# NethermindEth/zinc

Hardware: AMD Instinct MI355X
Metric: Zip commit+open MCoeffs/s at 2^24 witness (higher is better)
Workload: dtype i64

## Files before the change

zinc_amd/csrc/kernels_commit.cuh:

```cuda
#pragma once
#include <hip/hip_runtime.h>
#include <stdint.h>

#include "blake3.cuh"

namespace zipk {

typedef __int128 i128;
typedef unsigned __int128 u128;

#ifdef ZIPK_DEBUG_STAMPS
constexpr uint32_t kStampRec = 64;
__device__ __forceinline__ unsigned long long stamp_hw_id() {
    const uint32_t xcc = __builtin_amdgcn_s_getreg((3 << 11) | 20), hw = __builtin_amdgcn_s_getreg((31 << 11) | 4);
    return (unsigned long long)xcc | ((unsigned long long)hw << 8);
}
#endif

struct CommitArgs {
    const int64_t *evals;
    const uint32_t *perm1;
    const uint32_t *perm2;
    uint64_t *rows;
    uint32_t compact_rows;
// ... 121 lines not shown
    static constexpr bool MASKED = MODE != kStoreAll;
    uint32_t w0[E], w1[E], w2[E];
    const uint64_t *lz_lo = nullptr;
    const uint32_t *lz_hi = nullptr;
    uint32_t lz_stride = 0;
    template <int E0>
    __device__ __forceinline__ void entry(uint32_t &a, uint32_t &b, uint32_t &c) const {
        if (LAZY) {
            const uint64_t lo = lz_lo[E0 * lz_stride];
            a = (uint32_t)lo;
            b = (uint32_t)(lo >> 32);
            c = lz_hi[E0 * lz_stride];
        } else {
            a = w0[E0];
            b = w1[E0];
            c = w2[E0];
        }
    }
    uint64_t *out_row;
    uint32_t *tree;
    uint32_t cw, T, tid;
    uint32_t base = 0;
    uint32_t compact = 0;
    uint32_t smask = 0xFFFFFFFFu;
    static constexpr uint32_t NW = MODE == kStorePacked ? 32u : 8u;
    uint8_t *pk_v = nullptr, *pk_n = nullptr;
    uint32_t pk_off0 = 0, pk_off1 = 0, pk_off2 = 0;
    __device__ __forceinline__ void set_packed(const CommitArgs &a, uint32_t row) {
        uint8_t *g = a.pk + (size_t)(row >> 2) * 4 * a.pk_stride;
        pk_v = g + (row & 3u) * 16u;
        pk_n = g + (row & 3u) * 32u;
        pk_off0 = 4u * a.pk_off0;
        pk_off1 = 4u * a.pk_off1;
        pk_off2 = 4u * a.pk_off2;
    }
    uint32_t ptab[16] = {};
    template <int K>
    __device__ __forceinline__ uint32_t pbase() const { return (ptab[K >> 1] >> ((K & 1) * 16)) & 0xFFFFu; }
    static __device__ __forceinline__ uint32_t lanes_below(uint64_t m) {
        return __builtin_amdgcn_mbcnt_hi((uint32_t)(m >> 32), __builtin_amdgcn_mbcnt_lo((uint32_t)m, 0u));
    }
    template <int E0>
    __device__ __forceinline__ void store_row_of(uint32_t d0, uint32_t d1, uint32_t d2) {
        if (MASKED && !(smask & (1u << E0))) return;
        const uint32_t j = base + E0 * T + tid;
        const uint32_t s = (uint32_t)((int32_t)d2 >> 31);
        if (MODE == kStorePacked) {
            const uint32_t pos = pbase<E0>() + lanes_below(__builtin_amdgcn_ballot_w64(true));
            *reinterpret_cast<uint4 *>(pk_v + (size_t)pos * 64) = make_uint4(d0, d1, d2, s);
        } else if (compact) {
            *reinterpret_cast<uint4 *>(out_row + (size_t)j * 2) = make_uint4(d0, d1, d2, s);
        } else {
            uint4 *o = reinterpret_cast<uint4 *>(out_row + (size_t)j * 4);
            o[0] = make_uint4(d0, d1, d2, s);
            o[1] = make_uint4(s, s, s, s);
        }
    }
    template <int E0>
    __device__ __forceinline__ void store_row() {
        uint32_t d0, d1, d2;
        entry<E0>(d0, d1, d2);
        store_row_of<E0>(d0, d1, d2);
    }
    template <int E0>
    __device__ __forceinline__ void leaf(uint32_t (&h)[8]) {
        uint32_t d0, d1, d2;
        entry<E0>(d0, d1, d2);
        store_row_of<E0>(d0, d1, d2);
        blake3_leaf_sext96(d0, d1, d2, h);
        if (!MASKED || (smask & (0x100u << E0))) {
            if (MODE == kStorePacked) {
                const uint32_t pos = pbase<8 + E0>() + lanes_below(__builtin_amdgcn_ballot_w64(true));
                store_hash(reinterpret_cast<uint32_t *>(pk_n + pk_off0) + (size_t)pos * 32, h);
            } else {
                store_hash(tree + (size_t)(base + E0 * T + tid) * 8, h);
            }
        }
    }
    template <int LVL, int E0>
    __device__ __forceinline__ void store(const uint32_t (&h)[8]) {
        if (MASKED && LVL <= 2 && !(smask & ((LVL == 1 ? 0x10000u : 0x1000000u) << (E0 >> LVL)))) return;
        const uint32_t e = E0 + (tid & ((1u << LVL) - 1u));
        const uint32_t n = (base + e * T + tid) >> LVL;
        if (MODE == kStorePacked && LVL == 1) {
            const uint64_t act = __builtin_amdgcn_ballot_w64(true);
            const bool odd = tid & 1u;
            const uint32_t pos = (odd ? pbase<16 + (E0 >> 1) * 2 + 1>() : pbase<16 + (E0 >> 1) * 2>()) +
                                 lanes_below(act & (odd ? 0xAAAAAAAAAAAAAAAAull : 0x5555555555555555ull));
            store_hash(reinterpret_cast<uint32_t *>(pk_n + pk_off1) + (size_t)pos * 32, h);
        } else if (MODE == kStorePacked && LVL == 2) {
            const uint64_t act = __builtin_amdgcn_ballot_w64(true);
            const uint32_t q = tid & 3u;
            constexpr int K0 = 24 + ((E0 >> 2) & 1) * 4;
            const uint32_t b01 = (q & 1u) ? pbase<K0 + 1>() : pbase<K0>(), b23 = (q & 1u) ? pbase<K0 + 3>() : pbase<K0 + 2>();
            const uint32_t pos = ((q & 2u) ? b23 : b01) + lanes_below(act & (0x1111111111111111ull << q));
            store_hash(reinterpret_cast<uint32_t *>(pk_n + pk_off2) + (size_t)pos * 32, h);
        } else {
            store_hash(tree + ((size_t)level_off(cw, LVL) + n) * NW, h);
        }
    }
};

template <int E>
__device__ __forceinline__ uint32_t store_mask(const uint32_t *need, uint32_t cw, uint32_t base, uint32_t T, uint32_t tid) {
    if (!need) return 0xFFFFFFFFu;
    const uint32_t *nv = need, *n0 = nv + (cw + 31) / 32, *n1 = n0 + (cw + 31) / 32, *n2 = n1 + (cw / 2 + 31) / 32;
    uint32_t m = 0;
#pragma unroll
    for (int e = 0; e < E; e++) {
        const uint32_t j = base + e * T + tid;
        m |= ((nv[j >> 5] >> (j & 31)) & 1u) << e;
        m |= ((n0[j >> 5] >> (j & 31)) & 1u) << (8 + e);
    }
#pragma unroll
    for (int g = 0; g < E / 2; g++) {
        const uint32_t i = (base + (2 * g + (tid & 1u)) * T + tid) >> 1;
        m |= ((n1[i >> 5] >> (i & 31)) & 1u) << (16 + g);
    }
#pragma unroll
    for (int g = 0; g < E / 4; g++) {
        const uint32_t i = (base + (4 * g + (tid & 3u)) * T + tid) >> 2;
        m |= ((n2[i >> 5] >> (i & 31)) & 1u) << (24 + g);
    }
    return m;
}

template <int E, int E0, class Src>
__device__ __forceinline__ void store_rows_only(Src &src) {
    if constexpr (E0 < E) {
        src.template store_row<E0>();
        store_rows_only<E, E0 + 1>(src);
    }
}

template <int LVL, int E0, class Src>
__device__ __forceinline__ void bfly_hash(Src &src, uint32_t (&h)[8]) {
    if constexpr (LVL == 0) {
        src.template leaf<E0>(h);
    } else {
        uint32_t A[8], B[8], m[16];
        bfly_hash<LVL - 1, E0>(src, A);
        bfly_hash<LVL - 1, E0 + (1 << (LVL - 1))>(src, B);
        const bool up = (src.tid >> (LVL - 1)) & 1;
#pragma unroll
        for (int i = 0; i < 8; i++) {
            const uint32_t snd = up ? A[i] : B[i];
            const uint32_t rcv = __shfl_xor(snd, 1 << (LVL - 1), 64);
            m[i] = up ? rcv : A[i];
            m[8 + i] = up ? B[i] : rcv;
        }
        blake3_block64(m, h);
        src.template store<LVL, E0>(h);
    }
}

template <bool ILV>
__device__ __forceinline__ void upper_stage(const CommitArgs &a, uint32_t first, uint32_t nrows_c, uint32_t lvl, uint32_t nl,
                                            uint32_t lane, uint32_t nlanes) {
    constexpr uint32_t NW = kNodeWords<ILV>;
    const uint32_t cw = a.cw, depth = 31u - __builtin_clz(cw);
    const uint32_t u_shift = depth - (lvl - 1u) - nl;
    const uint32_t total = nrows_c << u_shift;
    const uint32_t slot0 = round_slot(blockIdx.x, gridDim.x, a.classes);
    for (uint32_t idx = lane; idx < total; idx += nlanes) {
        const uint32_t ri = idx >> u_shift, i = idx & ((1u << u_shift) - 1u);
        const uint32_t r = slot0 + (first + ri) * gridDim.x;
        uint32_t *tree = tree_of<ILV>(a.layers, cw, r);
        const uint32_t *ch = tree + ((size_t)level_off(cw, lvl - 1u) + ((size_t)i << nl)) * NW;
        uint32_t c0[8], c1[8], h0[8];
        load_hash(ch, c0);
        load_hash(ch + NW, c1);
        if (nl == 1u) {
            blake3_node(c0, c1, h0);
            store_hash(tree + ((size_t)level_off(cw, lvl) + i) * NW, h0);
            if (lvl == depth) store_hash(a.roots + (size_t)r * 8, h0);
        } else {
            uint32_t c2[8], c3[8], h1[8], h2[8];
            blake3_node(c0, c1, h0);
            uint32_t *o = tree + ((size_t)level_off(cw, lvl) + 2u * i) * NW;
            store_hash(o, h0);
            asm volatile("" ::: "memory");
            load_hash(ch + 2 * NW, c2);
            load_hash(ch + 3 * NW, c3);
            blake3_node(c2, c3, h1);
            store_hash(o + NW, h1);
            blake3_node(h0, h1, h2);
            store_hash(tree + ((size_t)level_off(cw, lvl + 1u) + i) * NW, h2);
            if (lvl + 1u == depth) store_hash(a.roots + (size_t)r * 8, h2);
        }
    }
}

struct ChunkCursor {
    uint32_t first = 0, index = 0;
    __device__ __forceinline__ bool ends_with(const CommitArgs &a, uint32_t round, bool last) const {
        if (last) return true;
        if (a.chunk_ends) return (a.chunk_ends >> round) & 1u;
        return (round + 1) % a.rounds_per_chunk == 0;
    }
    __device__ __forceinline__ void advance(uint32_t round) {
        first = round + 1;
        index++;
    }
};

constexpr uint32_t kFinisherFlagWords = 16;

template <bool HASH, bool ILV = false>
struct ChunkFinisher {
    bool pending = false;
    uint32_t p_first = 0, p_nrows = 0, p_lvl = 0, p_index = 0;
    uint32_t p_base = 0;
    uint32_t n_deferred = 0;
    uint32_t *flags = nullptr;

    __device__ __forceinline__ void init(uint32_t *lds_flags, uint32_t tid) {
        flags = lds_flags;
        if (tid < kFinisherFlagWords) lds_flags[tid] = 0;
    }

    __device__ __forceinline__ void top_of_row() const {
        if (HASH && pending) asm volatile("s_waitcnt vmcnt(0)" ::: "memory");
    }

    static __device__ __forceinline__ void publish(const CommitArgs &a, uint32_t index, uint32_t lane) {
        if (!a.chunk_done) return;
        asm volatile("s_waitcnt vmcnt(0)" ::: "memory");
        if (lane == 0) {
            __builtin_amdgcn_fence(__ATOMIC_RELEASE, "agent");
            asm volatile("s_waitcnt vmcnt(0)" ::: "memory");
            __hip_atomic_fetch_add(&a.chunk_done[index], 1u, __ATOMIC_RELAXED, __HIP_MEMORY_SCOPE_AGENT);
        }
    }

    static __device__ __forceinline__ void signal(uint32_t *flag, uint32_t lane) {
        asm volatile("s_waitcnt vmcnt(0)" ::: "memory");
        if (lane == 0) __hip_atomic_fetch_add(flag, 1u, __ATOMIC_RELEASE, __HIP_MEMORY_SCOPE_WORKGROUP);
    }
    static __device__ __forceinline__ void wait_for(uint32_t *flag, uint32_t target) {
        uint32_t spins = 0;
        while (__hip_atomic_load(flag, __ATOMIC_ACQUIRE, __HIP_MEMORY_SCOPE_WORKGROUP) < target) {
            __builtin_amdgcn_s_sleep(2);
            if (++spins > (1u << 24)) __builtin_trap();
        }
    }

    static __device__ __forceinline__ bool stage_wide(uint32_t cw, uint32_t lvl, uint32_t nl, uint32_t j) {
        return j == 0u || (cw >> (lvl - 1u + nl)) >= 64u;
    }
    static __device__ __forceinline__ uint32_t stage_waves(uint32_t cw, uint32_t depth, uint32_t lvl0, uint32_t j, uint32_t W) {
        const uint32_t lvl = lvl0 + 2u * j;
        if (lvl > depth) return 0u;
        return stage_wide(cw, lvl, depth - lvl >= 1u ? 2u : 1u, j) ? W : 1u;
    }
    __device__ __forceinline__ uint32_t target(uint32_t cw, uint32_t depth, uint32_t j, uint32_t W) const {
        return (n_deferred - 1u) * stage_waves(cw, depth, p_base, j, W) + stage_waves(cw, depth, p_lvl, j, W);
    }
    __device__ __forceinline__ void after_hash(const CommitArgs &a, uint32_t wave, uint32_t lane, uint32_t T) {
        if (!(HASH && pending)) return;
        pending = false;
        n_deferred++;
        constexpr uint32_t kFinWaves = 8u;
        const uint32_t W = T >= 64u * kFinWaves ? kFinWaves : T >= 256u ? 4u : (T + 63u) / 64u;
        if (wave >= W) return;
        const uint32_t cw = a.cw, depth = 31u - __builtin_clz(cw);
        uint32_t lvl = p_lvl, j = 0, owner = 0;
        bool wide = true;
        while (lvl <= depth) {
            const uint32_t nl = depth - lvl >= 1u ? 2u : 1u;
            wide = stage_wide(cw, lvl, nl, j);
            if (wide) {
                if (j) wait_for(flags + (j - 1u), target(cw, depth, j - 1u, W));
                upper_stage<ILV>(a, p_first, p_nrows, lvl, nl, lane + 64u * wave, 64u * W);
                signal(flags + j, lane);
            } else {
                owner = j % W;
                if (wave == owner) {
                    wait_for(flags + (j - 1u), target(cw, depth, j - 1u, W));
                    upper_stage<ILV>(a, p_first, p_nrows, lvl, nl, lane, 64u);
                    signal(flags + j, lane);
                }
            }
            lvl += nl;
            j++;
        }
        if (j == 0u || wide) owner = 0u;
        if (wave == owner) {
            if (j && wide) wait_for(flags + (j - 1u), target(cw, depth, j - 1u, W));
            publish(a, p_index, lane);
        }
    }

    __device__ __forceinline__ void after_loop(const CommitArgs &a, uint32_t wave, uint32_t lane, uint32_t T, unsigned char *lds,
                                               uint32_t lds_bytes) {
        if (!(HASH && pending)) return;
        __syncthreads();
        const uint32_t cw = a.cw, depth = 31u - __builtin_clz(cw);
        const uint32_t tid = lane + 64u * wave;
        const uint32_t w_in0 = cw >> (p_lvl - 1u);
        const uint32_t n_in0 = p_nrows * w_in0;
        if (p_lvl <= depth && (n_in0 + n_in0 / 2u) * 32u <= lds_bytes && n_in0 >= 2u) {
            constexpr uint32_t NW = kNodeWords<ILV>;
            pending = false;
            uint4 *bufA = reinterpret_cast<uint4 *>(lds), *bufB = bufA + 2u * n_in0;
            const uint32_t slot0 = round_slot(blockIdx.x, gridDim.x, a.classes);
            const uint32_t sh0 = 31u - __builtin_clz(w_in0);
            for (uint32_t idx = tid; idx < n_in0; idx += T) {
                const uint32_t ri = idx >> sh0, i = idx & (w_in0 - 1u);
                const uint32_t r = slot0 + (p_first + ri) * gridDim.x;
                const uint4 *src = reinterpret_cast<const uint4 *>(tree_of<ILV>(a.layers, cw, r) + ((size_t)level_off(cw, p_lvl - 1u) + i) * NW);
                bufA[2u * idx] = src[0];
                bufA[2u * idx + 1u] = src[1];
            }
            __syncthreads();
            uint4 *in = bufA, *out = bufB;
            for (uint32_t lvl = p_lvl; lvl <= depth; lvl++) {
                const uint32_t w = cw >> lvl, sh = 31u - __builtin_clz(w), m = p_nrows * w;
                for (uint32_t idx = tid; idx < m; idx += T) {
                    const uint32_t ri = idx >> sh, i = idx & (w - 1u);
                    const uint32_t r = slot0 + (p_first + ri) * gridDim.x;
                    const uint4 a0 = in[4u * idx], a1 = in[4u * idx + 1u], b0 = in[4u * idx + 2u], b1 = in[4u * idx + 3u];
                    const uint32_t c0[8] = {a0.x, a0.y, a0.z, a0.w, a1.x, a1.y, a1.z, a1.w};
                    const uint32_t c1[8] = {b0.x, b0.y, b0.z, b0.w, b1.x, b1.y, b1.z, b1.w};
                    uint32_t h[8];
                    blake3_node(c0, c1, h);
                    store_hash(tree_of<ILV>(a.layers, cw, r) + ((size_t)level_off(cw, lvl) + i) * NW, h);
                    if (lvl == depth) store_hash(a.roots + (size_t)r * 8, h);
                    out[2u * idx] = make_uint4(h[0], h[1], h[2], h[3]);
                    out[2u * idx + 1u] = make_uint4(h[4], h[5], h[6], h[7]);
                }
                __syncthreads();
                uint4 *t = in;
                in = out;
                out = t;
            }
            if (wave == 0u) publish(a, p_index, lane);
            return;
        }
        after_hash(a, wave, lane, T);
    }

    __device__ __forceinline__ void chunk_end(const CommitArgs &a, uint32_t first_level, const ChunkCursor &cc, uint32_t round,
                                              bool last, uint32_t tid, uint32_t T) {
        const uint32_t wave = __builtin_amdgcn_readfirstlane(tid >> 6), lane = tid & 63u;
        if (!HASH) {
            if (a.chunk_done) {
                __syncthreads();
                if (wave == 0) publish(a, cc.index, lane);
            }
            return;
        }
        const uint32_t cw = a.cw, depth = 31u - __builtin_clz(cw);
        const uint32_t first = cc.first, nrows_c = round - first + 1;
        uint32_t lvl = first_level;
        const bool now = last || lvl > depth;
        if (now) {
            __syncthreads();
            if (lvl <= depth) {
                const uint32_t nl = depth - lvl >= 1u ? 2u : 1u;
                upper_stage<ILV>(a, first, nrows_c, lvl, nl, tid, T);
                lvl += nl;
            }
        }
        if (depth == 0 && tid == 0) {
            for (uint32_t ri = 0; ri < nrows_c; ri++) {
                const uint32_t r = round_slot(blockIdx.x, gridDim.x, a.classes) + (first + ri) * gridDim.x;
                uint32_t h[8];
                load_hash(a.layers + (size_t)r * (2u * cw) * 8, h);
                store_hash(a.roots + (size_t)r * 8, h);
            }
        }
        if (!last) p_base = lvl;
        pending = true;
        p_first = first;
        p_nrows = nrows_c;
        p_lvl = lvl;
        p_index = cc.index;
    }
};

__device__ __forceinline__ void stamp_clock(const CommitArgs &a, int slot) {
    if (a.clock && blockIdx.x == 0 && threadIdx.x == 0) {
        a.clock[2 * slot] = __builtin_amdgcn_s_memtime();
        a.clock[2 * slot + 1] = __builtin_amdgcn_s_memrealtime();
    }
}

__device__ __forceinline__ uint32_t opaque_zero(uint32_t dep) {
    uint32_t z;
    asm volatile("s_mov_b32 %0, 0" : "=s"(z) : "s"(dep));
    return z;
}

template <int E, bool HASH, int MODE = kStoreAll>
__global__ void __launch_bounds__(1024, 4) raa_commit_kernel(CommitArgs a) {
    constexpr bool MASKED = MODE != kStoreAll;
    extern __shared__ __align__(16) unsigned char smem[];
    constexpr int LOGE = (E == 1) ? 0 : (E == 2) ? 1 : (E == 4) ? 2 : 3;
    static_assert((1 << LOGE) == E && E <= 8, "E must be 1, 2, 4 or 8");

    const uint32_t tid0 = threadIdx.x, T = blockDim.x;
    constexpr uint32_t PAD = 32 / E;
    const uint32_t PS = T + PAD;
    const uint32_t cw = a.cw, row_len = a.row_len;
    const bool active = tid0 < a.nact;
    stamp_clock(a, 0);

    i128 *wave_tot = reinterpret_cast<i128 *>(smem);
    uint64_t *t2lo = reinterpret_cast<uint64_t *>(smem + 512);
    uint32_t *t2hi = reinterpret_cast<uint32_t *>(t2lo + E * PS);
    int64_t *rowbuf = reinterpret_cast<int64_t *>(t2hi + E * PS);
    uint32_t pidx[E];
    auto load_pidx = [&](uint32_t t) {
#pragma unroll
        for (int e = 0; e < E; e++) {
            uint32_t v1 = 0, v2 = 0;
            if (active) {
                v1 = a.perm1[t * E + e] & (row_len - 1);
                const uint32_t p2 = a.perm2[t * E + e];
                v2 = (p2 & (E - 1)) * PS + (p2 >> LOGE);
            }
            pidx[e] = v1 | (v2 << 16);
        }
    };
    load_pidx(tid0);
    const uint32_t smask = (MASKED && active) ? store_mask<E>(a.need, cw, 0u, a.nact, tid0) : 0xFFFFFFFFu;
    uint32_t ptab[16] = {};
    if (MODE == kStorePacked) {
        const uint32_t *wt = a.pk_tab + (size_t)__builtin_amdgcn_readfirstlane(tid0 >> 6) * 16;
#pragma unroll
        for (int k = 0; k < 16; k++) ptab[k] = __builtin_amdgcn_readfirstlane(wt[k]);
    }
    constexpr int NPF = (E >= 2) ? E / 2 : 1;
    const bool prefetch = row_len == NPF * T;
    int64_t nxt[NPF];

#ifdef ZIPK_DEBUG_STAMPS
    unsigned long long ph_a = 0, ph_b = 0, ph_c = 0, ph_t;
    if (tid0 == 0 && a.stamps) {
        a.stamps[(size_t)kStampRec * blockIdx.x] = wall_clock64();
        a.stamps[(size_t)kStampRec * blockIdx.x + 2] = stamp_hw_id();
    }
#define ZIPK_PH(acc) do { const unsigned long long now_ = wall_clock64(); acc += now_ - ph_t; ph_t = now_; } while (0)
#else
#define ZIPK_PH(acc) do { } while (0)
#endif
    uint32_t round = 0;
    ChunkCursor cc;
    if (a.classes > 1u) {
        const uint32_t c = commit_class(blockIdx.x, gridDim.x, a.classes);
        cc.index = c;
        const uint32_t prio = (a.classes - 1u - c) * 3u / (a.classes - 1u);
        if (prio == 3u) __builtin_amdgcn_s_setprio(3);
        else if (prio == 2u) __builtin_amdgcn_s_setprio(2);
        else if (prio == 1u) __builtin_amdgcn_s_setprio(1);
    }
    ChunkFinisher<HASH, MODE == kStorePacked> fin;
    fin.init(reinterpret_cast<uint32_t *>(rowbuf + row_len), tid0);
    const uint32_t wave0 = __builtin_amdgcn_readfirstlane(tid0 >> 6);
    for (uint32_t row = round_slot(blockIdx.x, gridDim.x, a.classes); row < a.num_rows; row += gridDim.x, round++) {
#ifdef ZIPK_DEBUG_STAMPS
        ph_t = wall_clock64();
#endif
        const uint32_t z = opaque_zero(row);
        const uint32_t tid = tid0 + z;
        const int64_t *in = a.evals + (size_t)row * row_len;
        uint64_t *out_row = a.rows + (size_t)row * cw * (a.compact_rows ? 2 : 4);

        const bool has_next = row + gridDim.x < a.num_rows;
        if (!(prefetch && round)) {
            if (round) lds_barrier();
            for (uint32_t i = tid; i < row_len; i += T) rowbuf[i] = in[i];
            lds_barrier();
        }
        if (prefetch && has_next) {
            const int64_t *nin = a.evals + (size_t)(row + gridDim.x) * row_len;
#pragma unroll
            for (int k = 0; k < NPF; k++) nxt[k] = nin[k * T + tid];
        }

        i128 v[E];
        if (active) {
#pragma unroll
            for (int e = 0; e < E; e++) v[e] = (i128)rowbuf[(pidx[e] ^ z) & 0xFFFFu];
#pragma unroll
            for (int e = 1; e < E; e++) v[e] += v[e - 1];
        } else {
#pragma unroll
            for (int e = 0; e < E; e++) v[e] = 0;
        }
        {
            const i128 pre = block_exclusive_scan_i96(v[E - 1], wave_tot, 0);
            if (active) {
#pragma unroll
                for (int e = 0; e < E; e++) {
                    v[e] += pre;
                    const uint32_t slot = e * PS + tid;
                    t2lo[slot] = (uint64_t)v[e];
                    t2hi[slot] = (uint32_t)((u128)v[e] >> 64);
                }
            }
        }
        lds_barrier();
        if (active) {
#pragma unroll
            for (int e = 0; e < E; e++) {
                const uint32_t slot = (pidx[e] ^ z) >> 16;
                const uint64_t lo = t2lo[slot];
                const int64_t hi = (int64_t)(int32_t)t2hi[slot];
                v[e] = (i128)(((u128)(uint64_t)hi << 64) | lo);
            }
#pragma unroll
            for (int e = 1; e < E; e++) v[e] += v[e - 1];
        }
        {
            const i128 pre = block_exclusive_scan_i96(v[E - 1], wave_tot, 1);
#pragma unroll
            for (int e = 0; e < E; e++) v[e] += pre;
        }

        if (active) {
#pragma unroll
            for (int e = 0; e < E; e++) {
                const uint32_t slot = e * PS + tid;
                t2lo[slot] = (uint64_t)v[e];
                t2hi[slot] = (uint32_t)((u128)v[e] >> 64);
            }
        }
        if (prefetch && has_next) {
#pragma unroll
            for (int k = 0; k < NPF; k++) rowbuf[k * T + tid] = nxt[k];
        }
        fin.top_of_row();
        lds_barrier();
        ZIPK_PH(ph_a);
        if (active) {
            StridedLeaves<E, MODE, true> src;
            src.out_row = out_row;
            src.compact = a.compact_rows;
            src.tree = HASH ? tree_of<MODE == kStorePacked>(a.layers, cw, row) : nullptr;
            src.cw = cw;
            src.T = a.nact;
            src.tid = tid;
            src.smask = smask;
            if (MODE == kStorePacked) {
                src.set_packed(a, row);
#pragma unroll
                for (int k = 0; k < 16; k++) src.ptab[k] = ptab[k];
            }
            {
                const uint32_t slot0 = (tid & (E - 1)) * PS + (tid >> LOGE);
                src.lz_lo = t2lo + slot0;
                src.lz_hi = t2hi + slot0;
                src.lz_stride = a.nact >> LOGE;
            }
            if (HASH) {
                uint32_t top[8];
                bfly_hash<LOGE, 0>(src, top);
            } else {
                store_rows_only<E, 0>(src);
            }
        }
        ZIPK_PH(ph_b);
        fin.after_hash(a, wave0, tid0 & 63u, T);
        const bool last = row + gridDim.x >= a.num_rows;
        if (cc.ends_with(a, round, last)) {
            fin.chunk_end(a, LOGE + 1, cc, round, last, tid, T);
            cc.advance(round);
        }
        ZIPK_PH(ph_c);
#ifdef ZIPK_DEBUG_STAMPS
        if (tid0 == 0 && a.stamps && round < kStampRec - 8) a.stamps[(size_t)kStampRec * blockIdx.x + 8 + round] = ph_t;
#endif
    }
    fin.after_loop(a, wave0, tid0 & 63u, T, smem + 512, (uint32_t)(E * PS * 12u));
    stamp_clock(a, 1);
#ifdef ZIPK_DEBUG_STAMPS
    if (tid0 == 0 && a.stamps) {
        unsigned long long *o = a.stamps + (size_t)kStampRec * blockIdx.x;
        o[1] = wall_clock64();
        o[3] = ph_a; o[4] = ph_b; o[5] = ph_c; o[6] = round;
    }
#endif
}

constexpr size_t c16_lds_bytes(uint32_t T) {
    return 512 + (size_t)16 * (T + 2) * 8 + (size_t)16 * (T + 2) + (size_t)T * 4 + 64;
}

template <int B, int P = 0>
__device__ __forceinline__ void transpose8_stage(uint32_t (&x)[8], bool up) {
    if constexpr (P < 4) {
        constexpr int r = ((P >> B) << (B + 1)) | (P & ((1 << B) - 1)), r2 = r | (1 << B);
        const uint32_t lo = x[r], hi = x[r2];
        const uint32_t rcv = __shfl_xor(up ? lo : hi, 1 << B, 64);
        x[r] = up ? rcv : lo;
        x[r2] = up ? hi : rcv;
        transpose8_stage<B, P + 1>(x, up);
    }
}
__device__ __forceinline__ void transpose8(uint32_t (&x)[8], uint32_t lane) {
    transpose8_stage<0>(x, lane & 1u);
    transpose8_stage<1>(x, (lane >> 1) & 1u);
    transpose8_stage<2>(x, (lane >> 2) & 1u);
}

template <uint32_t T, bool HASH, int MODE = kStoreAll>
__global__ void __launch_bounds__(T, 4) raa_commit16_kernel(CommitArgs a) {
    constexpr bool MASKED = MODE != kStoreAll;
    static_assert(MODE == kStoreAll || MODE == kStoreHinted || MODE == kStorePacked, "store mode");
    extern __shared__ __align__(16) unsigned char smem[];
    constexpr int E = 16;
    constexpr uint32_t PS = T + 2;
    const uint32_t tid0 = threadIdx.x;
    const uint32_t cw = a.cw, row_len = a.row_len;
    stamp_clock(a, 0);

    i128 *wave_tot = reinterpret_cast<i128 *>(smem);
    uint64_t *t2lo = reinterpret_cast<uint64_t *>(smem + 512);
    int8_t *t2dh = reinterpret_cast<int8_t *>(t2lo + (size_t)E * PS);
    int32_t *ghi = reinterpret_cast<int32_t *>(t2dh + (size_t)E * PS);
    uint64_t *park_lo = reinterpret_cast<uint64_t *>(smem + 512);
    uint32_t *park_hi = reinterpret_cast<uint32_t *>(park_lo + (size_t)8 * PS);

    const uint32_t smask0 = MASKED ? store_mask<8>(a.need, cw, 0u, 16u, (tid0 & ~7u) * 16u + (tid0 & 7u)) : 0xFFFFFFFFu;
    const uint32_t smask1 = MASKED ? store_mask<8>(a.need, cw, 0u, 16u, (tid0 & ~7u) * 16u + 8u + (tid0 & 7u)) : 0xFFFFFFFFu;
    uint32_t ptab0[16] = {}, ptab1[16] = {};
    if (MODE == kStorePacked) {
        const uint32_t *wt = a.pk_tab + (size_t)__builtin_amdgcn_readfirstlane(tid0 >> 6) * 32;
#pragma unroll
        for (int k = 0; k < 16; k++) {
            ptab0[k] = __builtin_amdgcn_readfirstlane(wt[k]);
            ptab1[k] = __builtin_amdgcn_readfirstlane(wt[16 + k]);
        }
    }

    uint32_t round = 0;
    ChunkCursor cc;
    ChunkFinisher<HASH, MODE == kStorePacked> fin;
    fin.init(reinterpret_cast<uint32_t *>(ghi + T), tid0);
    const uint32_t wave0 = __builtin_amdgcn_readfirstlane(tid0 >> 6);
    for (uint32_t row = round_slot(blockIdx.x, gridDim.x, a.classes); row < a.num_rows; row += gridDim.x, round++) {
        fin.top_of_row();
        const uint32_t z = opaque_zero(row);
        const uint32_t tid = tid0 + z;
        const int64_t *in = a.evals + (size_t)row * row_len;
        uint64_t *out_row = a.rows + (size_t)row * cw * (a.compact_rows ? 2 : 4);

        uint32_t p2[E];
        i128 v[E];
        {
            const uint4 *q1 = reinterpret_cast<const uint4 *>(a.perm1 + (size_t)tid * E);
            const uint4 *q2 = reinterpret_cast<const uint4 *>(a.perm2 + (size_t)tid * E);
#pragma unroll
            for (int k = 0; k < E / 4; k++) {
                const uint4 s1 = q1[k], s2 = q2[k];
                v[4 * k + 0] = (i128)in[s1.x & (row_len - 1)];
                v[4 * k + 1] = (i128)in[s1.y & (row_len - 1)];
                v[4 * k + 2] = (i128)in[s1.z & (row_len - 1)];
                v[4 * k + 3] = (i128)in[s1.w & (row_len - 1)];
                p2[4 * k + 0] = s2.x;
                p2[4 * k + 1] = s2.y;
                p2[4 * k + 2] = s2.z;
                p2[4 * k + 3] = s2.w;
            }
        }
#pragma unroll
        for (int e = 1; e < E; e++) v[e] += v[e - 1];
        {
            const i128 pre = block_exclusive_scan_i96(v[E - 1], wave_tot, 0);
            const int32_t phi = (int32_t)(uint32_t)((u128)pre >> 64);
            ghi[tid] = phi;
#pragma unroll
            for (int e = 0; e < E; e++) {
                const i128 t = v[e] + pre;
                t2lo[e * PS + tid] = (uint64_t)t;
                t2dh[e * PS + tid] = (int8_t)((int32_t)(uint32_t)((u128)t >> 64) - phi);
            }
        }
        lds_barrier();
#pragma unroll
        for (int e = 0; e < E; e++) {
            const uint32_t j = p2[e];
            const uint32_t slot = (j & 15u) * PS + (j >> 4);
            const uint64_t lo = t2lo[slot];
            const int64_t hi = (int64_t)(ghi[j >> 4] + (int32_t)t2dh[slot]);
            v[e] = (i128)(((u128)(uint64_t)hi << 64) | lo);
        }
#pragma unroll
        for (int e = 1; e < E; e++) v[e] += v[e - 1];
        {
            const i128 pre = block_exclusive_scan_i96(v[E - 1], wave_tot, 1);
#pragma unroll
            for (int e = 0; e < E; e++) v[e] += pre;
        }
#pragma unroll
        for (int e = 8; e < E; e++) {
            park_lo[(e - 8) * PS + tid] = (uint64_t)v[e];
            park_hi[(e - 8) * PS + tid] = (uint32_t)((u128)v[e] >> 64);
        }
        uint32_t x0[8], x1[8], x2[8];
#pragma unroll
// ... 299 lines not shown
```

zinc_amd/csrc/zip_hip.hip:

```cpp
#include <hip/hip_runtime.h>
#include <dlfcn.h>
#include <algorithm>
#include <atomic>
#include <chrono>
#include <thread>

#include <climits>
#include <cstdarg>
#include <cstdio>
#include <cstdlib>
#include <cstring>
#include <functional>
#include <map>
#include <memory>
#include <mutex>
#include <new>
#include <string>
#include <vector>

#include "../../include/zip_hip.h"
#include "kernels_commit.cuh"
#include "kernels_open.cuh"
#include "kernels_verify.cuh"
#include "kernels_sumcheck.cuh"
// ... 609 lines not shown
    return 0;
}
void sub_limbs(uint64_t *a, const uint64_t *b, uint32_t n) {
    uint64_t borrow = 0;
    for (uint32_t i = 0; i < n; i++) {
        u128 d = (u128)a[i] - b[i] - borrow;
        a[i] = (uint64_t)d;
        borrow = (uint64_t)(d >> 64) & 1;
    }
}
void dbl_mod(uint64_t *x, const uint64_t *q, uint32_t n) {
    const uint64_t top = x[n - 1] >> 63;
    for (uint32_t i = n; i-- > 1;) x[i] = (x[i] << 1) | (x[i - 1] >> 63);
    x[0] <<= 1;
    if (top || cmp_limbs(x, q, n) >= 0) sub_limbs(x, q, n);
}

int32_t make_field_uncached(zip_ctx *ctx, const zip_field *zf, HostField *f);
int32_t make_field(zip_ctx *ctx, const zip_field *zf, HostField *f) {
    if (!zf) return fail(ctx, ZIP_ERR_NULL, "field is NULL");
    if (ctx && ctx->field_cache_valid && ctx->field_cache_in.limbs == zf->limbs &&
        !memcmp(ctx->field_cache_in.modulus, zf->modulus, 8 * (size_t)zf->limbs)) {
        memcpy(f, ctx->field_cache_out, sizeof(HostField));
        return ZIP_OK;
    }
    int32_t rc = make_field_uncached(ctx, zf, f);
    if (!rc && ctx) {
        ctx->field_cache_in = *zf;
        memcpy(ctx->field_cache_out, f, sizeof(HostField));
        ctx->field_cache_valid = true;
    }
    return rc;
}
int32_t make_field_uncached(zip_ctx *ctx, const zip_field *zf, HostField *f) {
    if (!zf) return fail(ctx, ZIP_ERR_NULL, "field is NULL");
    if (zf->limbs < 2 || zf->limbs > 4)
        return fail(ctx, ZIP_ERR_UNSUPPORTED, "field limbs %u not in {2,3,4}", zf->limbs);
    if (!(zf->modulus[0] & 1)) return fail(ctx, ZIP_ERR_INVALID_PARAM, "modulus must be odd");
    const uint32_t n = f->fl = zf->limbs;
    bool gt1 = zf->modulus[0] > 1;
    for (uint32_t i = 1; i < n; i++) gt1 |= zf->modulus[i] != 0;
    if (!gt1) return fail(ctx, ZIP_ERR_INVALID_PARAM, "modulus must be > 1");
    memcpy(f->modulus, zf->modulus, 8 * n);
    uint64_t inv = 1;
    for (int i = 0; i < 63; i++) {
        inv *= inv;
        inv *= f->modulus[0];
    }
    f->inv = (uint64_t)0 - inv;
    uint64_t x[8] = {1};
    for (uint32_t i = 0; i < 64 * n; i++) dbl_mod(x, f->modulus, n);
    memcpy(f->r, x, 8 * n);
    for (uint32_t i = 0; i < 64 * n; i++) dbl_mod(x, f->modulus, n);
    memcpy(f->r2, x, 8 * n);
    f->quirk_mod = 0;
    if (f->modulus[n - 1] >> 63) {
        uint64_t m[8] = {0};
        sub_limbs(m, f->modulus, n);
        bool small = true;
        for (uint32_t i = 1; i < n; i++) small &= (m[i] == 0);
        if (small) f->quirk_mod = m[0];
    }
    return ZIP_OK;
}

template <int FL>
FieldDev<FL> to_dev(const HostField &h) {
    FieldDev<FL> d;
    for (int i = 0; i < FL; i++) {
        d.modulus[i] = h.modulus[i];
        d.r2[i] = h.r2[i];
    }
    d.inv = h.inv;
    return d;
}

int32_t ensure_dynamic_lds(zip_ctx *ctx, const void *kern, size_t bytes) {
    static std::mutex mu;
    static std::map<std::pair<const void *, int>, size_t> granted;
    std::lock_guard<std::mutex> g(mu);
    size_t &have = granted[std::make_pair(kern, ctx->device)];
    if (bytes > have) {
        HIP_TRY(ctx, hipFuncSetAttribute(kern, hipFuncAttributeMaxDynamicSharedMemorySize, (int)bytes));
        have = bytes;
    }
    return ZIP_OK;
}

template <int E, bool HASH, int MODE = kStoreAll>
int32_t launch_commit(zip_ctx *ctx, const CommitArgs &a, uint32_t threads, uint32_t grid, hipStream_t st) {
    size_t lds = 512 + (size_t)E * (threads + 32 / E) * 12 + (size_t)a.row_len * 8 + 4 * kFinisherFlagWords;
    auto kern = raa_commit_kernel<E, HASH, MODE>;
    if (int32_t rc = ensure_dynamic_lds(ctx, reinterpret_cast<const void *>(kern), lds)) return rc;
    LaunchTimer t(ctx, HASH ? "raa_commit_kernel" : "raa_encode_kernel", st);
    hipLaunchKernelGGL(kern, dim3(grid), dim3(threads), lds, st, a);
    HIP_TRY(ctx, hipGetLastError());
    return ZIP_OK;
}

template <bool HASH, int MODE = kStoreAll>
int32_t launch_commit16(zip_ctx *ctx, const CommitArgs &a, uint32_t grid, hipStream_t st) {
    constexpr uint32_t T = 1024;
    auto kern = raa_commit16_kernel<T, HASH, MODE>;
    if (int32_t rc = ensure_dynamic_lds(ctx, reinterpret_cast<const void *>(kern), c16_lds_bytes(T))) return rc;
    LaunchTimer t(ctx, HASH ? "raa_commit_kernel" : "raa_encode_kernel", st);
    hipLaunchKernelGGL(kern, dim3(grid), dim3(T), c16_lds_bytes(T), st, a);
    HIP_TRY(ctx, hipGetLastError());
    return ZIP_OK;
}

template <bool HASH>
int32_t launch_commit_slab(zip_ctx *ctx, const CommitArgs &a, uint32_t grid, hipStream_t st) {
    auto kern = a.cw == 65536 ? raa_commit_slab_kernel<64, HASH> : raa_commit_slab_kernel<32, HASH>;
    if (int32_t rc = ensure_dynamic_lds(ctx, reinterpret_cast<const void *>(kern), cslab_lds_bytes())) return rc;
    LaunchTimer t(ctx, HASH ? "raa_commit_kernel" : "raa_encode_kernel", st);
    hipLaunchKernelGGL(kern, dim3(grid), dim3(kSlabThreads), cslab_lds_bytes(), st, a);
    HIP_TRY(ctx, hipGetLastError());
    return ZIP_OK;
}

struct CommitGeom {
    uint32_t e, threads;
    size_t lds;
};
CommitGeom commit_geom(uint32_t cw, uint32_t row_len) {
    CommitGeom g{};
    if (cw >= 32768) { g.e = cw / kSlabThreads; g.threads = kSlabThreads; g.lds = cslab_lds_bytes(); return g; }
    if (cw == 16384) { g.e = 16; g.threads = 1024; g.lds = c16_lds_bytes(1024); return g; }
    if (cw >= 512) { g.e = 8; g.threads = cw / 8; }
    else if (cw == 256) { g.e = 4; g.threads = 64; }
    else if (cw == 128) { g.e = 2; g.threads = 64; }
    else { g.e = 1; g.threads = 64; }
    g.lds = 512 + (size_t)g.e * (g.threads + 32 / g.e) * 12 + (size_t)row_len * 8 + 4 * kFinisherFlagWords;
    return g;
}
uint32_t commit_wgs_per_cu(const CommitGeom &g) {
    if (g.e > 16) return 1;
    uint32_t by_threads = 2048 / g.threads, by_lds = (uint32_t)((160u * 1024u) / g.lds);
    uint32_t k = by_threads < by_lds ? by_threads : by_lds;
    if (k > 8) k = 8;
    return k ? k : 1;
}

bool commit_supports_hint(uint32_t cw) { return cw >= 512 && cw <= 16384; }
constexpr uint32_t kRingSlots = 64, kRingChunks = 16, kRingStride = 16;
constexpr size_t kHintTables = 8192, kHintBytes = kHintTables + 8 * (8192 / 32) + 4 * 4096 + 64, kPackedRanksAt = kHintTables + 2048;
static bool packed_enabled() {
    return env_long("ZIP_HIP_PACKED", 1, 0, 1) != 0;
}
static void plan_packed(HintPlan &P) {
    const uint32_t cw = P.cw, wv = (cw + 31) / 32, w1 = (cw / 2 + 31) / 32;
    const uint32_t *sec[4] = {P.bm.data(), P.bm.data() + wv, P.bm.data() + 2 * wv, P.bm.data() + 2 * wv + w1};
    const uint32_t bits[4] = {cw, cw, cw / 2, cw / 4};
    const uint32_t waves = P.threads / 64, phases = P.e == 16 ? 2 : 1, sT = P.e == 16 ? 16 : P.threads;
    for (int k = 0; k < 4; k++) P.pos[k].assign(bits[k], 0xFFFF);
    P.wave_tab.assign((size_t)waves * phases * 16, 0);
    uint32_t cnt[4] = {0, 0, 0, 0};
    auto member = [&](int k, uint32_t i) { return (sec[k][i >> 5] >> (i & 31u)) & 1u; };
    for (uint32_t w = 0; w < waves; w++)
        for (uint32_t q = 0; q < phases; q++) {
            uint16_t base[32];
            auto stid = [&](uint32_t l) {
                const uint32_t tid = 64 * w + l;
                return P.e == 16 ? (tid & ~7u) * 16u + q * 8u + (tid & 7u) : tid;
            };
            auto site = [&](int k, int slot, uint32_t step, uint32_t shift, uint32_t cls, uint32_t ncls) {
                base[slot] = (uint16_t)cnt[k];
                for (uint32_t l = cls; l < 64; l += ncls) {
                    const uint32_t i = (step * sT + stid(l)) >> shift;
                    if (member(k, i)) P.pos[k][i] = (uint16_t)cnt[k]++;
                }
            };
            for (uint32_t e = 0; e < 8; e++) site(0, (int)e, e, 0, 0, 1);
            for (uint32_t e = 0; e < 8; e++) site(1, (int)(8 + e), e, 0, 0, 1);
            for (uint32_t g = 0; g < 4; g++)
                for (uint32_t par = 0; par < 2; par++) site(2, (int)(16 + 2 * g + par), 2 * g + par, 1, par, 2);
            for (uint32_t g = 0; g < 2; g++)
                for (uint32_t c4 = 0; c4 < 4; c4++) site(3, (int)(24 + 4 * g + c4), 4 * g + c4, 2, c4, 4);
            uint32_t *tab = P.wave_tab.data() + ((size_t)w * phases + q) * 16;
            for (uint32_t k = 0; k < 16; k++) tab[k] = (uint32_t)base[2 * k] | ((uint32_t)base[2 * k + 1] << 16);
        }
    uint32_t at = (cnt[0] * 16u + 127u) & ~127u;
    P.L.off[0] = at;
    at = (at + cnt[1] * 32u + 127u) & ~127u;
    P.L.off[1] = at;
    at = (at + cnt[2] * 32u + 127u) & ~127u;
    P.L.off[2] = at;
    at = (at + cnt[3] * 32u + 127u) & ~127u;
    P.L.stride = at;
}
static std::shared_ptr<HintPlan> get_hint_plan(zip_ctx *ctx, const uint32_t *cols, uint32_t n_cols, bool want_packed) {
    const uint32_t cw = ctx->p.codeword_len;
    const CommitGeom g = commit_geom(cw, ctx->p.row_len);
    if (ctx->hint_plan) {
        const HintPlan &h = *ctx->hint_plan;
        if (h.cw == cw && h.e == g.e && h.threads == g.threads && h.want_packed == want_packed && h.cols.size() == n_cols &&
            (n_cols == 0 || !memcmp(h.cols.data(), cols, (size_t)n_cols * 4)))
            return ctx->hint_plan;
    }
    auto P = std::make_shared<HintPlan>();
    P->cw = cw;
    P->e = g.e;
    P->threads = g.threads;
    P->want_packed = want_packed;
    P->cols.assign(cols, cols + n_cols);
    const uint32_t wv = (cw + 31) / 32, w1 = (cw / 2 + 31) / 32, w2 = (cw / 4 + 31) / 32;
    P->bm.assign(2 * (size_t)wv + w1 + w2, 0);
    uint32_t *nv = P->bm.data(), *n0 = nv + wv, *n1 = n0 + wv, *n2 = n1 + w1;
    for (uint32_t i = 0; i < n_cols; i++) {
        const uint32_t col = cols[i];
        nv[col >> 5] |= 1u << (col & 31);
        const uint32_t s0 = col ^ 1u, s1 = (col >> 1) ^ 1u, s2 = (col >> 2) ^ 1u;
        n0[s0 >> 5] |= 1u << (s0 & 31);
        n1[s1 >> 5] |= 1u << (s1 & 31);
        n2[s2 >> 5] |= 1u << (s2 & 31);
    }
    if (want_packed && n_cols && (g.e == 8 || g.e == 16) && cw >= 512 && g.threads % 64 == 0 && cw == g.e * g.threads &&
        ctx->depth >= 3) {
        plan_packed(*P);
        P->own_ranks.resize((size_t)n_cols * 4);
        P->packed = P->L.stride > 0 && P->wave_tab.size() * 4 <= kPackedRanksAt - kHintTables &&
                    kPackedRanksAt + P->own_ranks.size() * 2 <= kHintBytes && P->ranks(cols, n_cols, P->own_ranks.data());
    }
    std::vector<unsigned char> img(kHintBytes, 0);
    memcpy(img.data(), P->bm.data(), P->bm.size() * 4);
    size_t used = P->bm.size() * 4;
    if (P->packed) {
        memcpy(img.data() + kHintTables, P->wave_tab.data(), P->wave_tab.size() * 4);
        memcpy(img.data() + kPackedRanksAt, P->own_ranks.data(), P->own_ranks.size() * 2);
        used = kPackedRanksAt + P->own_ranks.size() * 2;
    }
    void *blk = nullptr;
    if (used <= kHintBytes && pool_alloc(ctx, kHintBytes, &blk) == ZIP_OK) {
        if (hipMemcpy(blk, img.data(), used, hipMemcpyHostToDevice) == hipSuccess) {
            P->dev = static_cast<unsigned char *>(blk);
            std::shared_ptr<bool> alive = ctx->alive;
            P->release = [ctx, alive](unsigned char *p) { if (*alive) pool_release(ctx, p); };
        } else {
            pool_release(ctx, blk);
            (void)hipGetLastError();
        }
    }
    ctx->hint_plan = P;
    return P;
}

template <bool HASH>
int32_t dispatch_commit(zip_ctx *ctx, CommitArgs a, uint32_t grid, hipStream_t st) {
    const CommitGeom g = commit_geom(a.cw, a.row_len);
    a.nact = a.cw / g.e < g.threads ? a.cw / g.e : g.threads;
    if (HASH && a.need) {
        if (g.e == 8 && a.pk) return launch_commit<8, HASH, HASH ? kStorePacked : kStoreAll>(ctx, a, g.threads, grid, st);
        if (g.e == 16 && a.pk) return launch_commit16<HASH, HASH ? kStorePacked : kStoreAll>(ctx, a, grid, st);
        a.pk = nullptr;
        if (g.e == 16) return launch_commit16<HASH, HASH ? kStoreHinted : kStoreAll>(ctx, a, grid, st);
        if (g.e == 8) return launch_commit<8, HASH, HASH ? kStoreHinted : kStoreAll>(ctx, a, g.threads, grid, st);
        a.need = nullptr;
    }
    a.pk = nullptr;
    switch (g.e) {
        case 64:
        case 32: return launch_commit_slab<HASH>(ctx, a, grid, st);
        case 16: return launch_commit16<HASH>(ctx, a, grid, st);
        case 8: return launch_commit<8, HASH>(ctx, a, g.threads, grid, st);
        case 4: return launch_commit<4, HASH>(ctx, a, g.threads, grid, st);
        case 2: return launch_commit<2, HASH>(ctx, a, g.threads, grid, st);
        default: return launch_commit<1, HASH>(ctx, a, g.threads, grid, st);
    }
}

template <int NL>
int32_t launch_upper(zip_ctx *ctx, hipStream_t st, uint32_t *layers, uint32_t *roots, uint32_t trees, uint32_t cw,
                     uint32_t level_in, uint32_t depth) {
    const uint64_t total = (uint64_t)trees * ((cw >> level_in) >> NL);
    const uint32_t threads = 256;
    const uint32_t blocks = (uint32_t)((total + threads - 1) / threads);
    LaunchTimer t(ctx, "merkle_upper_kernel", st);
    hipLaunchKernelGGL(merkle_upper_kernel<NL>, dim3(blocks), dim3(threads), 0, st, layers, roots, trees, cw,
                       level_in, depth);
    HIP_TRY(ctx, hipGetLastError());
    return ZIP_OK;
}

int32_t merkle_upper_levels(zip_ctx *ctx, hipStream_t st, uint32_t *layers, uint32_t *roots, uint32_t trees,
                            uint32_t cw, uint32_t level, uint32_t depth) {
    if (depth == 0) {
        LaunchTimer t(ctx, "copy_roots_depth0_kernel", st);
        hipLaunchKernelGGL(copy_roots_depth0_kernel, dim3((trees + 255) / 256), dim3(256), 0, st, layers, roots,
                           trees, cw);
        HIP_TRY(ctx, hipGetLastError());
        return ZIP_OK;
    }
    while (level < depth) {
        const uint32_t rem = depth - level;
        int32_t rc;
        if (rem >= 4) {
            rc = launch_upper<4>(ctx, st, layers, roots, trees, cw, level, depth);
            level += 4;
        } else if (rem == 3) {
            rc = launch_upper<3>(ctx, st, layers, roots, trees, cw, level, depth);
            level += 3;
        } else if (rem == 2) {
            rc = launch_upper<2>(ctx, st, layers, roots, trees, cw, level, depth);
            level += 2;
        } else {
            rc = launch_upper<1>(ctx, st, layers, roots, trees, cw, level, depth);
            level += 1;
        }
        if (rc) return rc;
    }
    return ZIP_OK;
}

int32_t stage_evals(zip_ctx *ctx, const int64_t *evals, zip_mem_kind kind, size_t n, Scratch &tmp,
                    const int64_t **dev) {
    if (!evals) return fail(ctx, ZIP_ERR_NULL, "evals is NULL");
    if (kind == ZIP_MEM_DEVICE) {
        *dev = evals;
        return ZIP_OK;
    }
    int32_t rc = tmp.get(n * 8);
    if (rc) return rc;
    if ((rc = copy_h2d_bounced(ctx, tmp.ptr, evals, n * 8, ctx->stream))) return rc;
    *dev = tmp.as<int64_t>();
    return ZIP_OK;
}

struct CombineOut {
    uint64_t *uprime = nullptr;
    uint64_t *row_limbs = nullptr;
    uint8_t *row_be = nullptr;
};

struct CombineScratch {
    Scratch pint, pa, pb;
    explicit CombineScratch(zip_ctx *c) : pint(c), pa(c), pb(c) {}
};

template <int FL>
int32_t run_combine_fl(zip_ctx *ctx, const int64_t *evals_d, const int64_t *coeffs_dv,
                       const uint64_t *q0_dv, const HostField *hf, bool do_int, bool do_field, const CombineOut &out,
                       CombineScratch *ext, int phase) {
    const uint32_t R = ctx->rows_local, C = ctx->p.row_len;
    const uint32_t bx = (C + 255) / 256;
    uint32_t chunks = 512 / bx;
    if (chunks > 32) chunks = 32;
    if (chunks < 1) chunks = 1;
    if (chunks > R) chunks = R;
    const uint32_t rpc = (R + chunks - 1) / chunks;
    chunks = (R + rpc - 1) / rpc;

    const hipStream_t st = ctx->stream;
    CombineScratch own(ctx);
    CombineScratch &cs = ext ? *ext : own;
    Scratch &pint = cs.pint, &pa = cs.pa, &pb = cs.pb;
    int32_t rc;
    CombineArgs a{};
    a.evals = evals_d;
    a.num_rows = R;
    a.row_len = C;
    a.rows_per_chunk = rpc;
    a.prio = 1;
    a.quirk_mod = hf ? hf->quirk_mod : 0;
    if (do_int) {
        if (phase != 2 && (rc = pint.get((size_t)chunks * C * 3 * 8))) return rc;
        a.coeffs = coeffs_dv;
        a.part_int = pint.as<uint64_t>();
    }
    if (do_field) {
        if (phase != 2 && (rc = pa.get((size_t)chunks * C * (FL + 2) * 8))) return rc;
        a.q0 = q0_dv;
        a.part_a = pa.as<uint64_t>();
    }
    if (phase != 2 && (rc = pb.get((size_t)chunks * (FL + 3) * 8))) return rc;
    a.part_k = pb.as<uint64_t>();
    if (phase != 2) {
        LaunchTimer t(ctx, "combine_rows_kernel", st);
        const dim3 grid(bx, chunks), block(256);
        if (a.quirk_mod && do_field) {
            if (do_int)
                hipLaunchKernelGGL((combine_rows_kernel<FL, true, true, true>), grid, block, 0, st, a);
            else
                hipLaunchKernelGGL((combine_rows_kernel<FL, false, true, true>), grid, block, 0, st, a);
        } else if (do_int && do_field)
            hipLaunchKernelGGL((combine_rows_kernel<FL, true, true, false>), grid, block, 0, st, a);
        else if (do_int)
            hipLaunchKernelGGL((combine_rows_kernel<FL, true, false, false>), grid, block, 0, st, a);
        else
            hipLaunchKernelGGL((combine_rows_kernel<FL, false, true, false>), grid, block, 0, st, a);
        HIP_TRY(ctx, hipGetLastError());
    }
    FinalizeArgs fa{};
    fa.part_int = a.part_int;
    fa.part_a = a.part_a;
    fa.part_k = a.part_k;
    fa.num_rows = R;
    fa.chunks = chunks;
    fa.row_len = C;
    fa.m_limbs = ctx->p.m_limbs;
    fa.prio = a.prio;
    fa.uprime = out.uprime;
    fa.row_limbs = out.row_limbs;
    fa.row_be = out.row_be;
    FieldDev<FL> fd{};
// ... 3023 lines not shown
```

Before: 11320.

## Hash packed E=8 commit leaves in-lane and drop the final LDS barrier

For the packed E=8 hashing commit path, each thread now hashes its own eight contiguous leaves (a subtree kept inside the lane) instead of butterfly-shuffling strided leaves across lanes. Because every thread reads only the LDS slots it wrote itself, the barrier after the scan write-back is removed and the prefetch store is moved ahead of the scan. The host hint-plan builder is changed so packed positions follow the new per-thread site order, and a guard rejects configurations where not all threads are active. The cost is that the top levels now rely on global tree stores instead of cross-lane shuffles, and packed-store ranks use ballot/mbcnt per site.

```diff
diff --git a/zinc_amd/csrc/kernels_commit.cuh b/zinc_amd/csrc/kernels_commit.cuh
--- a/zinc_amd/csrc/kernels_commit.cuh
+++ b/zinc_amd/csrc/kernels_commit.cuh
@@ -297,6 +297,81 @@
         blake3_block64(m, h);
         src.template store<LVL, E0>(h);
     }
+}
+
+struct InLaneLeaves {
+    static constexpr uint32_t NW = 32u;
+    const uint64_t *lz_lo = nullptr;
+    const uint32_t *lz_hi = nullptr;
+    uint32_t lz_stride = 0;
+    uint32_t *tree = nullptr;
+    uint32_t cw = 0, tid = 0;
+    uint32_t smask = 0;
+    uint8_t *pk_v = nullptr, *pk_n = nullptr;
+    uint32_t pk_off0 = 0, pk_off1 = 0, pk_off2 = 0;
+    __device__ __forceinline__ void set_packed(const CommitArgs &a, uint32_t row) {
+        uint8_t *g = a.pk + (size_t)(row >> 2) * 4 * a.pk_stride;
+        pk_v = g + (row & 3u) * 16u;
+        pk_n = g + (row & 3u) * 32u;
+        pk_off0 = 4u * a.pk_off0;
+        pk_off1 = 4u * a.pk_off1;
+        pk_off2 = 4u * a.pk_off2;
+    }
+    static constexpr int kSites = 22;
+    uint32_t ptab[kSites / 2] = {};
+    template <int K>
+    __device__ __forceinline__ uint32_t pbase() const { return (ptab[K >> 1] >> ((K & 1) * 16)) & 0xFFFFu; }
+    template <int K>
+    __device__ __forceinline__ uint32_t rank() const {
+        const uint64_t m = __builtin_amdgcn_ballot_w64(true);
+        return pbase<K>() + __builtin_amdgcn_mbcnt_hi((uint32_t)(m >> 32), __builtin_amdgcn_mbcnt_lo((uint32_t)m, 0u));
+    }
+    template <int E0>
+    __device__ __forceinline__ void leaf(uint32_t (&h)[8]) {
+        const uint64_t lo = lz_lo[E0 * lz_stride];
+        const uint32_t d0 = (uint32_t)lo, d1 = (uint32_t)(lo >> 32), d2 = lz_hi[E0 * lz_stride];
+        if (smask & (1u << E0)) {
+            const uint32_t s = (uint32_t)((int32_t)d2 >> 31);
+            *reinterpret_cast<uint4 *>(pk_v + (size_t)rank<E0>() * 64) = make_uint4(d0, d1, d2, s);
+        }
+        blake3_leaf_sext96(d0, d1, d2, h);
+        if (smask & (0x100u << E0)) store_hash(reinterpret_cast<uint32_t *>(pk_n + pk_off0) + (size_t)rank<8 + E0>() * 32, h);
+    }
+    __device__ __forceinline__ void store(int LVL, int g, const uint32_t (&h)[8]) {
+        if (LVL == 1) {
+            if (!(smask & (0x10000u << g))) return;
+            const uint32_t pos = g == 0 ? rank<16>() : g == 1 ? rank<17>() : g == 2 ? rank<18>() : rank<19>();
+            store_hash(reinterpret_cast<uint32_t *>(pk_n + pk_off1) + (size_t)pos * 32, h);
+        } else if (LVL == 2) {
+            if (!(smask & (0x1000000u << g))) return;
+            const uint32_t pos = g == 0 ? rank<20>() : rank<21>();
+            store_hash(reinterpret_cast<uint32_t *>(pk_n + pk_off2) + (size_t)pos * 32, h);
+        } else {
+            store_hash(tree + ((size_t)level_off(cw, 3) + tid) * NW, h);
+        }
+    }
+};
+
+__device__ __forceinline__ uint32_t store_mask_inlane(const uint32_t *need, uint32_t cw, uint32_t tid) {
+    const uint32_t *nv = need, *n0 = nv + (cw + 31) / 32, *n1 = n0 + (cw + 31) / 32, *n2 = n1 + (cw / 2 + 31) / 32;
+    uint32_t m = 0;
+#pragma unroll
+    for (int e = 0; e < 8; e++) {
+        const uint32_t j = tid * 8u + e;
+        m |= ((nv[j >> 5] >> (j & 31)) & 1u) << e;
+        m |= ((n0[j >> 5] >> (j & 31)) & 1u) << (8 + e);
+    }
+#pragma unroll
+    for (int g = 0; g < 4; g++) {
+        const uint32_t i = tid * 4u + g;
+        m |= ((n1[i >> 5] >> (i & 31)) & 1u) << (16 + g);
+    }
+#pragma unroll
+    for (int g = 0; g < 2; g++) {
+        const uint32_t i = tid * 2u + g;
+        m |= ((n2[i >> 5] >> (i & 31)) & 1u) << (24 + g);
+    }
+    return m;
 }
 
 template <bool ILV>
@@ -540,6 +615,8 @@
 template <int E, bool HASH, int MODE = kStoreAll>
 __global__ void __launch_bounds__(1024, 4) raa_commit_kernel(CommitArgs a) {
     constexpr bool MASKED = MODE != kStoreAll;
+    constexpr bool INLANE = MODE == kStorePacked;
+    static_assert(!INLANE || (E == 8 && HASH), "packed commits: the 8-entry hashing kernel");
     extern __shared__ __align__(16) unsigned char smem[];
     constexpr int LOGE = (E == 1) ? 0 : (E == 2) ? 1 : (E == 4) ? 2 : 3;
     static_assert((1 << LOGE) == E && E <= 8, "E must be 1, 2, 4 or 8");
@@ -569,12 +646,15 @@
         }
     };
     load_pidx(tid0);
-    const uint32_t smask = (MASKED && active) ? store_mask<E>(a.need, cw, 0u, a.nact, tid0) : 0xFFFFFFFFu;
-    uint32_t ptab[16] = {};
-    if (MODE == kStorePacked) {
+    const uint32_t smask = !(MASKED && active) ? 0xFFFFFFFFu
+                           : INLANE            ? store_mask_inlane(a.need, cw, tid0)
+                                               : store_mask<E>(a.need, cw, 0u, a.nact, tid0);
+    constexpr int NPT = InLaneLeaves::kSites / 2;
+    uint32_t ptab[NPT] = {};
+    if constexpr (INLANE) {
         const uint32_t *wt = a.pk_tab + (size_t)__builtin_amdgcn_readfirstlane(tid0 >> 6) * 16;
 #pragma unroll
-        for (int k = 0; k < 16; k++) ptab[k] = __builtin_amdgcn_readfirstlane(wt[k]);
+        for (int k = 0; k < NPT; k++) ptab[k] = __builtin_amdgcn_readfirstlane(wt[k]);
     }
     constexpr int NPF = (E >= 2) ? E / 2 : 1;
     const bool prefetch = row_len == NPF * T;
@@ -658,6 +738,14 @@
 #pragma unroll
             for (int e = 1; e < E; e++) v[e] += v[e - 1];
         }
+        auto under_last_barrier = [&]() {
+            if (prefetch && has_next) {
+#pragma unroll
+                for (int k = 0; k < NPF; k++) rowbuf[k * T + tid] = nxt[k];
+            }
+            fin.top_of_row();
+        };
+        if constexpr (INLANE) under_last_barrier();
         {
             const i128 pre = block_exclusive_scan_i96(v[E - 1], wave_tot, 1);
 #pragma unroll
@@ -672,14 +760,28 @@
                 t2hi[slot] = (uint32_t)((u128)v[e] >> 64);
             }
         }
-        if (prefetch && has_next) {
-#pragma unroll
-            for (int k = 0; k < NPF; k++) rowbuf[k * T + tid] = nxt[k];
-        }
-        fin.top_of_row();
-        lds_barrier();
+        if constexpr (INLANE) {
+            asm volatile("" ::: "memory");
+        } else {
+            under_last_barrier();
+            lds_barrier();
+        }
         ZIPK_PH(ph_a);
-        if (active) {
+        if constexpr (INLANE) {
+            InLaneLeaves src;
+            src.lz_lo = t2lo + tid;
+            src.lz_hi = t2hi + tid;
+            src.lz_stride = PS;
+            src.tree = tree_of<true>(a.layers, cw, row);
+            src.cw = cw;
+            src.tid = tid;
+            src.smask = smask;
+            src.set_packed(a, row);
+#pragma unroll
+            for (int k = 0; k < NPT; k++) src.ptab[k] = ptab[k];
+            uint32_t top[8];
+            subtree_hash<LOGE, 0>(src, top);
+        } else if (active) {
             StridedLeaves<E, MODE, true> src;
             src.out_row = out_row;
             src.compact = a.compact_rows;
@@ -688,11 +790,6 @@
             src.T = a.nact;
             src.tid = tid;
             src.smask = smask;
-            if (MODE == kStorePacked) {
-                src.set_packed(a, row);
-#pragma unroll
-                for (int k = 0; k < 16; k++) src.ptab[k] = ptab[k];
-            }
             {
                 const uint32_t slot0 = (tid & (E - 1)) * PS + (tid >> LOGE);
                 src.lz_lo = t2lo + slot0;
diff --git a/zinc_amd/csrc/zip_hip.hip b/zinc_amd/csrc/zip_hip.hip
--- a/zinc_amd/csrc/zip_hip.hip
+++ b/zinc_amd/csrc/zip_hip.hip
@@ -785,31 +785,45 @@
     const uint32_t cw = P.cw, wv = (cw + 31) / 32, w1 = (cw / 2 + 31) / 32;
     const uint32_t *sec[4] = {P.bm.data(), P.bm.data() + wv, P.bm.data() + 2 * wv, P.bm.data() + 2 * wv + w1};
     const uint32_t bits[4] = {cw, cw, cw / 2, cw / 4};
-    const uint32_t waves = P.threads / 64, phases = P.e == 16 ? 2 : 1, sT = P.e == 16 ? 16 : P.threads;
+    const uint32_t waves = P.threads / 64, phases = P.e == 16 ? 2 : 1;
     for (int k = 0; k < 4; k++) P.pos[k].assign(bits[k], 0xFFFF);
     P.wave_tab.assign((size_t)waves * phases * 16, 0);
     uint32_t cnt[4] = {0, 0, 0, 0};
     auto member = [&](int k, uint32_t i) { return (sec[k][i >> 5] >> (i & 31u)) & 1u; };
     for (uint32_t w = 0; w < waves; w++)
         for (uint32_t q = 0; q < phases; q++) {
-            uint16_t base[32];
-            auto stid = [&](uint32_t l) {
-                const uint32_t tid = 64 * w + l;
-                return P.e == 16 ? (tid & ~7u) * 16u + q * 8u + (tid & 7u) : tid;
-            };
-            auto site = [&](int k, int slot, uint32_t step, uint32_t shift, uint32_t cls, uint32_t ncls) {
-                base[slot] = (uint16_t)cnt[k];
-                for (uint32_t l = cls; l < 64; l += ncls) {
-                    const uint32_t i = (step * sT + stid(l)) >> shift;
-                    if (member(k, i)) P.pos[k][i] = (uint16_t)cnt[k]++;
-                }
-            };
-            for (uint32_t e = 0; e < 8; e++) site(0, (int)e, e, 0, 0, 1);
-            for (uint32_t e = 0; e < 8; e++) site(1, (int)(8 + e), e, 0, 0, 1);
-            for (uint32_t g = 0; g < 4; g++)
-                for (uint32_t par = 0; par < 2; par++) site(2, (int)(16 + 2 * g + par), 2 * g + par, 1, par, 2);
-            for (uint32_t g = 0; g < 2; g++)
-                for (uint32_t c4 = 0; c4 < 4; c4++) site(3, (int)(24 + 4 * g + c4), 4 * g + c4, 2, c4, 4);
+            uint16_t base[32] = {};
+            if (P.e == 8) {
+                auto own_site = [&](int k, int slot, uint32_t per, uint32_t g) {
+                    base[slot] = (uint16_t)cnt[k];
+                    for (uint32_t l = 0; l < 64; l++) {
+                        const uint32_t i = (64 * w + l) * per + g;
+                        if (member(k, i)) P.pos[k][i] = (uint16_t)cnt[k]++;
+                    }
+                };
+                for (uint32_t e = 0; e < 8; e++) own_site(0, (int)e, 8, e);
+                for (uint32_t e = 0; e < 8; e++) own_site(1, (int)(8 + e), 8, e);
+                for (uint32_t g = 0; g < 4; g++) own_site(2, (int)(16 + g), 4, g);
+                for (uint32_t g = 0; g < 2; g++) own_site(3, (int)(20 + g), 2, g);
+            } else {
+                auto stid = [&](uint32_t l) {
+                    const uint32_t tid = 64 * w + l;
+                    return (tid & ~7u) * 16u + q * 8u + (tid & 7u);
+                };
+                auto site = [&](int k, int slot, uint32_t step, uint32_t shift, uint32_t cls, uint32_t ncls) {
+                    base[slot] = (uint16_t)cnt[k];
+                    for (uint32_t l = cls; l < 64; l += ncls) {
+                        const uint32_t i = (step * 16u + stid(l)) >> shift;
+                        if (member(k, i)) P.pos[k][i] = (uint16_t)cnt[k]++;
+                    }
+                };
+                for (uint32_t e = 0; e < 8; e++) site(0, (int)e, e, 0, 0, 1);
+                for (uint32_t e = 0; e < 8; e++) site(1, (int)(8 + e), e, 0, 0, 1);
+                for (uint32_t g = 0; g < 4; g++)
+                    for (uint32_t par = 0; par < 2; par++) site(2, (int)(16 + 2 * g + par), 2 * g + par, 1, par, 2);
+                for (uint32_t g = 0; g < 2; g++)
+                    for (uint32_t c4 = 0; c4 < 4; c4++) site(3, (int)(24 + 4 * g + c4), 4 * g + c4, 2, c4, 4);
+            }
             uint32_t *tab = P.wave_tab.data() + ((size_t)w * phases + q) * 16;
             for (uint32_t k = 0; k < 16; k++) tab[k] = (uint32_t)base[2 * k] | ((uint32_t)base[2 * k + 1] << 16);
         }
@@ -883,6 +897,7 @@
     const CommitGeom g = commit_geom(a.cw, a.row_len);
     a.nact = a.cw / g.e < g.threads ? a.cw / g.e : g.threads;
     if (HASH && a.need) {
+        if (g.e == 8 && a.pk && a.nact != g.threads) return ZIP_ERR_INVALID_PARAM;
         if (g.e == 8 && a.pk) return launch_commit<8, HASH, HASH ? kStorePacked : kStoreAll>(ctx, a, g.threads, grid, st);
         if (g.e == 16 && a.pk) return launch_commit16<HASH, HASH ? kStorePacked : kStoreAll>(ctx, a, grid, st);
         a.pk = nullptr;
```

Result: faster. 11600 (median of 6 runs) (+2.4%).
